# Niema-Lab/AmpliPy

Measured on AMD Instinct MI355X. Metric: aligned reads/s through trim+pileup+call, 30 kb ref @ 10k x depth, higher is better.
Workload: dtype u8/int32

## Files before the change

amplipy_amd/csrc/amp_fast.hpp:

```cpp
#pragma once

#include "amp_tile.hpp"
#include "amp_bf.hpp"

namespace amp {

#ifndef AMP_F_LDSPAD
#define AMP_F_LDSPAD 0
#endif
#ifndef AMP_F4_LEAN
#define AMP_F4_LEAN 1
#endif
#ifndef AMP_F4_BF
#define AMP_F4_BF 1
#endif
__device__ __forceinline__ Bf bf_of(const Cig2 &s) { return Bf{s.a, s.m1, s.k, s.m2, s.c, s.kind, s.op, s.punt ? 1u : 0u}; }
__device__ __forceinline__ Cig2 cig2_of(const Bf &b) { return Cig2{b.op, b.a, b.m1, b.k, b.m2, b.c, b.kind, b.punt != 0u}; }
constexpr int F_NP = 10;
constexpr int F_MAXLEN = 152;
constexpr int F_PW = 256;
#ifndef AMP_F_REPS
#define AMP_F_REPS 8
#endif
constexpr int F_REP = AMP_F_REPS;
// ... 198 lines not shown
    const uint32_t se1 = __builtin_amdgcn_perm(0x00000010u, 0x00080018u, (sq.y >> 4) & 0x07070707u);
    const uint32_t so1 = __builtin_amdgcn_perm(0x00000010u, 0x00080018u, sq.y & 0x07070707u);
    const uint32_t f0 = nibble_to_bytes(m, 0), f1 = nibble_to_bytes(m, 1), f2 = nibble_to_bytes(m, 2), f3 = nibble_to_bytes(m, 3);
    const uint32_t wb = wrep + (inwin ? (uint32_t)d0 * 4u + (((uint32_t)d0 & 1u) ? ooff : 0u) : 0u);
#define F_SH(d, sh, js, v, jv) "v_lshlrev_b32_sdwa " d ", " sh ", " v " dst_sel:DWORD dst_unused:UNUSED_PAD src0_sel:BYTE_" #js " src1_sel:BYTE_" #jv "\n\t"
#define F_AQ(t, off) "ds_add_u64 %0, " t " offset:" #off "\n\t"
    asm volatile(F_SH("v252", "%1", 0, "%5", 0) F_SH("v253", "%2", 0, "%5", 1) F_AQ("v[252:253]", 0)
                 F_SH("v254", "%1", 1, "%5", 2) F_SH("v255", "%2", 1, "%5", 3) F_AQ("v[254:255]", 8)
                 F_SH("v252", "%1", 2, "%6", 0) F_SH("v253", "%2", 2, "%6", 1) F_AQ("v[252:253]", 16)
                 F_SH("v254", "%1", 3, "%6", 2) F_SH("v255", "%2", 3, "%6", 3) F_AQ("v[254:255]", 24)
                 F_SH("v252", "%3", 0, "%7", 0) F_SH("v253", "%4", 0, "%7", 1) F_AQ("v[252:253]", 32)
                 F_SH("v254", "%3", 1, "%7", 2) F_SH("v255", "%4", 1, "%7", 3) F_AQ("v[254:255]", 40)
                 F_SH("v252", "%3", 2, "%8", 0) F_SH("v253", "%4", 2, "%8", 1) F_AQ("v[252:253]", 48)
                 F_SH("v254", "%3", 3, "%8", 2) F_SH("v255", "%4", 3, "%8", 3) "ds_add_u64 %0, v[254:255] offset:56"
                 : : "v"(wb), "v"(se0), "v"(so0), "v"(se1), "v"(so1), "v"(f0), "v"(f1), "v"(f2), "v"(f3) : "memory", "v252", "v253", "v254", "v255");
#undef F_SH
#undef F_AQ
    return redo ? 1u : 0u;
}
__device__ __forceinline__ uint32_t range_bits16(int32_t klo, int32_t khi) {
    klo = klo < 0 ? 0 : (klo > 16 ? 16 : klo); khi = khi > 16 ? 16 : (khi < 0 ? 0 : khi);
    return ((1u << khi) - 1u) & ~((1u << klo) - 1u);
}

#if defined(AMP_DEV) && (!defined(AMP_ABL) || defined(AMP_ABL_STAMPS))
#define F_DBG_PARAM , uint32_t *f_dbg
#define F_GLOB ++f_glob
#define F_EPIW(k) do { __builtin_amdgcn_s_waitcnt(0x4F74); f_epw[0] = wall_clock64(); __builtin_amdgcn_s_waitcnt(0x0F7A); f_epw[1] = wall_clock64(); __builtin_amdgcn_s_waitcnt(0); f_ep[k] = wall_clock64(); } while (0)
#define F_EPI(k) do { __builtin_amdgcn_s_waitcnt(0); f_ep[k] = wall_clock64(); } while (0)
#define F_DBG_ARG(x) , (x)
#define F_STAMP_DECL unsigned long long f_t[8] = {0, 0, 0, 0, 0, 0, 0, 0}, f_prev = __builtin_amdgcn_s_memtime(); const unsigned long long f_k0 = f_prev, f_w0 = wall_clock64(); unsigned long long f_ep[3] = {0, 0, 0}, f_epw[2] = {0, 0}; uint32_t f_glob = 0
#define F_STAMP(k) do { __builtin_amdgcn_sched_barrier(0); __builtin_amdgcn_s_waitcnt(0xC07F); unsigned long long f_n = __builtin_amdgcn_s_memtime(); f_t[k] += f_n - f_prev; f_prev = f_n; __builtin_amdgcn_sched_barrier(0); } while (0)
#define F_STAMP_VM(k) do { __builtin_amdgcn_sched_barrier(0); __builtin_amdgcn_s_waitcnt(0x0070); unsigned long long f_n = __builtin_amdgcn_s_memtime(); f_t[k] += f_n - f_prev; f_prev = f_n; __builtin_amdgcn_sched_barrier(0); } while (0)
#define F_STAMP_OUT do { f_t[0] = __builtin_amdgcn_s_memtime() - f_k0; const unsigned long long f_w1 = wall_clock64(); f_t[7] = f_w1 - f_w0; if (lane == 0) { for (int k = 0; k < 8; ++k) atomicAdd(&ctr[CTR_PHASE0 + k], f_t[k]); \
    atomicMax(&ctr[CTR_STAMP0], f_t[7]); atomicMax(&ctr[CTR_STAMP0 + 1], ~f_t[7]); atomicMax(&ctr[CTR_STAMP0 + 2], ~f_w0); atomicMax(&ctr[CTR_STAMP0 + 3], f_w1); \
    if (f_dbg && wave == 0) { uint32_t *f_o = f_dbg + blockIdx.x * 8; f_o[0] = (uint32_t)f_t[7]; f_o[1] = (uint32_t)f_w0; for (int k = 1; k < 7; ++k) f_o[1 + k] = (uint32_t)(f_t[k] >> 4); } \
    if (f_dbg) { uint32_t *f_o = f_dbg + F_DBG_WAVE0 + (blockIdx.x * F_WAVES + wave) * F_DBG_WAVEWORDS; f_o[0] = (uint32_t)((f_t[1] + f_t[2] + f_t[3] + f_t[4] + f_t[5] + f_t[6]) >> 4); f_o[1] = (uint32_t)(f_epw[0] - f_w0); f_o[2] = (uint32_t)(f_epw[1] - f_epw[0]); f_o[3] = (uint32_t)(f_ep[0] - f_epw[1]); f_o[4] = (uint32_t)(f_ep[1] - f_ep[0]); f_o[5] = (uint32_t)(f_ep[2] - f_ep[1]); } } } while (0)
#else
#define F_DBG_PARAM
#define F_DBG_ARG(x)
#define F_GLOB
#define F_EPIW(k)
#define F_EPI(k)
#define F_STAMP_DECL
#define F_STAMP(k)
#define F_STAMP_VM(k)
#define F_STAMP_OUT
#endif

#define F_ARGS \
    const int32_t *a_pos, int32_t a_min_quality, const uint16_t *a_flag, int32_t a_window, const int32_t *a_tlen, int32_t a_do_trim, \
    const uint32_t *a_lseq, int32_t a_do_count, const uint32_t *a_cig_off32, int32_t a_ref_len, const uint32_t *a_cig, int32_t a_max_primer_len, \
    const uint32_t *a_seq_off8, int32_t reads_per_block, const uint8_t *a_seq, int32_t a_epoch, const uint8_t *a_qual, int32_t pad1, \
    const int32_t *a_min_start, int32_t pad2, const int32_t *a_max_end, int32_t pad3, \
    int32_t *a_new_pos, int32_t pad4, uint32_t *a_new_ncig, int32_t pad5, uint32_t *a_new_cig, int32_t pad6, int32_t *a_o_ref_len, int32_t pad7, \
    uint8_t *a_trim_flags, int32_t pad8, uint8_t *a_status, int32_t pad9, \
    uint32_t *counts, int32_t pad10, amp_ins_event *a_ev, int32_t pad11, unsigned long long *a_ctr, int32_t pad12, uint32_t *a_ins_at, int32_t pad13, \
    uint32_t *glist, int32_t pad14, uint32_t *gcnt, int32_t pad15, \
    int64_t a_n_reads, int32_t pad17, uint64_t read_base, int32_t pad18, long long a_ev_cap
#define F_ARGS_PASS(P, rd, out, eb, rpb) \
    (rd).pos, (P).min_quality, (rd).flag, (P).window, (rd).tlen, (P).do_trim, (rd).lseq, (P).do_count, (rd).cig_off32, (P).ref_len, (rd).cig, \
    (P).max_primer_len, (rd).seq_off8, (rpb), (rd).seq, (int32_t)(P).epoch, (rd).qual, 0, (P).min_start, 0, (P).max_end, 0, (out).new_pos, 0, (out).new_ncig, 0, \
    (out).new_cig, 0, (out).ref_len, 0, (out).trim_flags, 0, (out).status, 0, counts, 0, (eb).ev, 0, (eb).ctr, 0, (eb).ins_at, 0, glist, 0, gcnt, 0, \
    (rd).n_reads, 0, read_base, 0, (eb).cap

#if AMP_F_ADD64
#define F_COUNT5(sq, m, d0, lim, wr) count_piece5q(sq, m, d0, lim, wr, (uint32_t)(F_REPW * 4))
#else
#define F_COUNT5(sq, m, d0, lim, wr) count_piece5(sq, m, d0, lim, wr)
#endif
template <int W>
__global__ void __launch_bounds__(F_WAVES * 64, 2)
k_fast(F_ARGS F_DBG_PARAM) {
    const KParams P{a_min_quality, a_window, a_do_trim, a_do_count, a_ref_len, a_max_primer_len, a_min_start, a_max_end, (uint32_t)a_epoch};
    const amp_dev_reads rd{a_n_reads, a_pos, a_flag, a_tlen, a_lseq, a_cig_off32, a_cig, a_seq_off8, a_seq, a_qual, 0, 0};
    const DevOut out{a_new_pos, a_new_ncig, a_new_cig, a_o_ref_len, a_trim_flags, a_status};
    const EventBuf eb{a_ev, a_ctr, a_ins_at, a_ev_cap};
    __shared__ uint4 s_stage[F_WAVES][(F_PAD + F_STAGE + 16) / 16];
    __shared__ __attribute__((aligned(8))) uint32_t s_pwin[F_WAVES][F_REP * F_REPW];
    __shared__ uint32_t s_bwin[F_BPL * F_BW];
    __shared__ uint32_t s_ticket, s_gcur;
#if AMP_F_LDSPAD > 0
    __shared__ uint32_t s_pad[AMP_F_LDSPAD / 4];
    if (P.ref_len == -12345) s_pad[threadIdx.x] = 1;
#endif
    unsigned long long *const ctr = eb.ctr;
    const int tid = threadIdx.x, wave = tid >> 6, lane = tid & 63;
    F_STAMP_DECL;
    const int64_t n = rd.n_reads;
    const int64_t rb = (int64_t)blockIdx.x * reads_per_block;
    const int64_t re = rb + reads_per_block < n ? rb + reads_per_block : n;
    lds_u32 *const bwin = (lds_u32 *)s_bwin;
    lds_u32 *const pwin = (lds_u32 *)s_pwin[wave];
    for (int i = tid; i < F_BPL * F_BW; i += F_WAVES * 64) bwin[i] = 0;
    for (int i = lane; i < F_REP * F_REPW; i += 64) pwin[i] = 0;
    if (lane < F_PAD / 4) ((lds_u32 *)s_stage[wave])[lane] = 0x11111111u;
    if (tid == 0) { s_ticket = 0; s_gcur = 0; }
    if (tid == 0 && blockIdx.x == 0) { eb.ctr[CTR_LONG_N] = 0ull; eb.ctr[CTR_LONG_TICKET] = 0ull; eb.ctr[CTR_GEN_LEFT] = 0ull; }
    int32_t bw_base = rb < n ? rd.pos[rb] : 0;
    bw_base = (bw_base < 16 ? 0 : bw_base - 16) & ~15;
    __syncthreads();

    const int32_t mq = P.min_quality;
    const uint32_t mqc = (uint32_t)(mq > 256 ? 256 : mq);
    const uint32_t thr = mqc * (uint32_t)W;
    const uint32_t mqb = (uint32_t)mq * 0x01010101u;
    const uint32_t G = (uint32_t)P.ref_len;
    const uint32_t n_tb = re > rb ? (uint32_t)((re - rb + 63) / 64) : 0u;
    auto take_ticket = [&]() {
        uint32_t t = 0;
        if (lane == 0) t = __hip_atomic_fetch_add((lds_u32 *)&s_ticket, 1u, __ATOMIC_RELAXED, __HIP_MEMORY_SCOPE_WORKGROUP);
        return (uint32_t)__builtin_amdgcn_readfirstlane((int)t);
    };
    const int64_t wend = re;
    unsigned long long n_err = 0;
#ifndef AMP_F_REPSHIFT
#define AMP_F_REPSHIFT 2
#endif
    const uint32_t rep = (F_REP & (F_REP - 1)) ? ((uint32_t)lane >> AMP_F_REPSHIFT) % (uint32_t)F_REP : ((uint32_t)lane >> AMP_F_REPSHIFT) & (uint32_t)(F_REP - 1);
    const uint32_t phi_lane = ((uint32_t)lane >> 1) & 1u ? 8u : 0u;
#if AMP_F_ADD64
    lds_u8 *const wrep = (lds_u8 *)pwin + (rep & (uint32_t)(F_REP / 2 - 1)) * (uint32_t)(2 * F_REPW * 4);
    static_assert((F_REP & 1) == 0 && (F_REPW & 1) == 1, "two arrays per replica, the second one an odd number of words behind the first");
#else
    lds_u8 *const wrep = (lds_u8 *)pwin + rep * (uint32_t)(F_REPW * 4);
#endif
    lds_u8 *const stage = (lds_u8 *)s_stage[wave] + F_PAD;
    int32_t pw_base = 0;
    int pw_tiles = F_FLUSH;
    const unsigned ev_shard = blockIdx.x & (EV_SHARDS - 1);
    amp_ins_event *const ev_list = eb.ev + (size_t)ev_shard * (size_t)eb.cap;
    unsigned long long ev_base = 0;
    uint32_t ev_left = 0;

    auto fold = [&]() {
        asm volatile("s_waitcnt lgkmcnt(0)" ::: "memory");
        wave_sync();
#pragma unroll 1
        for (int idx = lane; idx < F_PW; idx += 64) {
            uint32_t ag = 0, ct = 0;
#pragma unroll
            for (int r = 0; r < F_REP; ++r) {
                const uint32_t w = pwin[r * F_REPW + idx];
                pwin[r * F_REPW + idx] = 0;
                ag += w & 0x00FF00FFu; ct += (w >> 8) & 0x00FF00FFu;
            }
            if (ag | ct) {
                const int32_t p = pw_base + idx;
                const uint32_t d = (uint32_t)(p - bw_base);
                const uint32_t c4[4] = {ag & 0xFFFFu, ct & 0xFFFFu, ag >> 16, ct >> 16};
#pragma unroll
                for (int c = 0; c < 4; ++c) {
                    if (!c4[c]) continue;
                    if (d < (uint32_t)F_BW) lds_add(bwin + c * F_BW + d, c4[c]);
                    else if ((uint32_t)p < G) { atomicAdd(&counts[(size_t)p * AMP_NSYM + c], c4[c]); F_GLOB; }
                }
            }
        }
        wave_sync();
    };
    auto pad_events = [&]() {
        if ((uint32_t)lane < ev_left && (long long)(ev_base + (unsigned)lane) < eb.cap) ev_list[ev_base + (unsigned)lane] = amp_ins_event{-1, 0u, 0, 0};
    };

    struct Hdr { int32_t pos, tlen; uint32_t lseq, flag, c0, c1, o8; };
    struct HdrP { int32_t pos; uint32_t lf, c0, o8;
        __device__ uint32_t lseq() const { return lf & 0xFFFFu; }
        __device__ uint32_t nops() const { return (lf >> 19) & 7u; }
        __device__ uint32_t flag() const { return ((lf >> 16) & 1u) | (((lf >> 17) & 1u) << 4); }
        __device__ bool isize_flag() const { return (lf >> 18) & 1u; } };
    auto pack_hdr = [&](const Hdr &h) {
        const uint32_t n = h.c1 - h.c0, at = (uint32_t)(h.tlen < 0 ? -(int64_t)h.tlen : (int64_t)h.tlen);
        const bool isz = ((int64_t)at - P.max_primer_len) > (int64_t)h.lseq;
        return HdrP{h.pos, (h.lseq > 0xFFFFu ? 0xFFFFu : h.lseq) | ((h.flag & 1u) << 16) | (((h.flag >> 4) & 1u) << 17) | ((isz ? 1u : 0u) << 18) | ((n > 7u ? 7u : n) << 19),
                    h.c0, h.o8};
    };
    struct Cg { uint32_t w[5]; };
    struct Geo { uint32_t np, phi, row, Tq; int ntake; bool solo, taken, fastq; };
    struct Tabs { int32_t L, R; };
    struct Bytes { uint4 raws[F_STAGE / 2048]; };
    struct Shape { Cig2 s; bool ok; int32_t refspan; };
    auto load_hdr = [&](int64_t t0) {
        Hdr h{0, 0, 0u, 0u, 0u, 0u, 0u};
        const int64_t i = t0 + lane;
        if (i < wend) {
            h.pos = rd.pos[i]; h.flag = rd.flag[i]; h.tlen = rd.tlen[i]; h.lseq = rd.lseq[i];
            h.c0 = rd.cig_off32[i]; h.c1 = rd.cig_off32[i + 1]; h.o8 = rd.seq_off8[i];
        }
        return h;
    };
    auto load_cig = [&](const HdrP &h) {
        Cg c{{0u, 0u, 0u, 0u, 0u}};
        const uint32_t nops = h.nops();
        if (nops >= 1u && nops <= 5u) {
#pragma unroll
            for (uint32_t k = 0; k < 5u; ++k) c.w[k] = rd.cig[h.c0 + (k < nops ? k : 0u)];
        }
        return c;
    };
    auto geometry = [&](const HdrP &h, int64_t t0, uint32_t &m0) {
        Geo g;
        const bool valid = t0 + lane < wend;
        const uint32_t hl = h.lseq();
        const bool shortq = valid && hl >= 1u && hl <= (uint32_t)F_MAXLEN;
        g.phi = shortq ? phi_lane : 0u;
        g.np = shortq ? (hl + g.phi + 15u) >> 4 : 1u;
        m0 = __builtin_amdgcn_readfirstlane(h.o8);
        g.row = (h.o8 - m0) * 8u;
        const uint32_t nch = (hl + 7u) >> 3;
        const bool fits = valid && h.o8 >= m0 && (h.o8 - m0) <= (uint32_t)(F_STAGE / 8) &&
                          g.row + 8u * nch + (shortq ? 8u : 0u) <= (uint32_t)F_STAGE;
        const unsigned long long fitmask = __ballot(fits);
        g.ntake = fitmask == ~0ull ? 64 : __builtin_ctzll(~fitmask);
        g.solo = g.ntake == 0;
        if (g.solo) g.ntake = 1;
        g.taken = lane < g.ntake && !g.solo;
        g.Tq = g.solo ? 0u : (uint32_t)__builtin_amdgcn_readlane((int)(g.row + 8u * nch), g.ntake - 1);
        g.fastq = g.taken && shortq;
        return g;
    };
    auto shape_of = [&](const HdrP &h, const Cg &c, bool fastq) {
        Shape r;
#if AMP_F4_BF
        bool ok;
        r.s = cig2_of(bf_from_words5((int)h.nops(), c.w[0], c.w[1], c.w[2], c.w[3], c.w[4], (int32_t)h.lseq(), F_MAXINS, F_MAXDEL, ok));
        r.ok = ok & fastq;
        if (!r.ok) r.s = Cig2{0u, 0, 0, 0, 0, 0, 0, false};
#else
        r.s = Cig2{0u, 0, 0, 0, 0, 0, 0, false};
        const int nops = (int)h.nops();
        r.ok = fastq && nops >= 1 && nops <= 5 && cig2_from_words5(nops, c.w, (int32_t)h.lseq(), r.s);
        if (r.ok && ((r.s.kind == 1 && r.s.k > F_MAXINS) || (r.s.kind == 2 && r.s.k > F_MAXDEL))) r.ok = false;
        if (!r.ok) r.s = Cig2{0u, 0, 0, 0, 0, 0, 0, false};
#endif
        r.refspan = r.ok ? r.s.m1 + r.s.m2 + (r.s.kind == 2 ? r.s.k : 0) : 1;
        return r;
    };
    auto load_tabs = [&](const HdrP &h, const Shape &sh) {
        Tabs t{-1, -1};
        const bool in_ref = (uint32_t)h.pos < G && (uint32_t)(h.pos + sh.refspan - 1) < G;
        if (sh.ok && P.do_trim && in_ref) { t.L = P.max_end[h.pos]; t.R = P.min_start[h.pos + sh.refspan - 1]; }
        return t;
    };
    auto issue_bytes = [&](const Geo &g, uint32_t m0) {
        Bytes x;
        const uint8_t *qrun = rd.qual + (int64_t)m0 * 8;
        const uint8_t *srun = rd.seq + (int64_t)m0 * 4;
        const uint32_t lastq = g.Tq ? (g.Tq - 1u) & ~15u : 0u, lasts = g.Tq ? ((g.Tq >> 1) - 1u) & ~15u : 0u;
#pragma unroll
        for (int sl = 0; sl < F_STAGE / 1024; ++sl) {
            uint32_t off = (uint32_t)(sl * 1024 + lane * 16);
            off = off < lastq ? off : lastq;
            __builtin_amdgcn_global_load_lds((const __attribute__((address_space(1))) void *)(qrun + off),
                                             (__attribute__((address_space(3))) void *)(stage + sl * 1024), 16, 0, 0);
        }
#pragma unroll
        for (int sl = 0; sl < F_STAGE / 2048; ++sl) {
            uint32_t off = (uint32_t)(sl * 1024 + lane * 16);
            off = off < lasts ? off : lasts;
            const uint32_t *sp = (const uint32_t *)(srun + off);
            x.raws[sl] = make_uint4(sp[0], sp[1], sp[2], sp[3]);
        }
        return x;
    };
    enum : uint32_t { P_STORED = 1u << 24, P_LIST = 1u << 25, P_STATUS_ONLY = 1u << 26 };
    struct Pend { uint32_t i, slot_lo; int32_t pos, reflen; uint32_t meta, cw0, cw1, cw2, cw3, cw4; };
    Pend pend{0u, 0u, 0, 0, 0u, 0u, 0u, 0u, 0u, 0u};
    auto store_pending = [&](const Pend &r) {
#if defined(AMP_DEV) && defined(AMP_ABL)
        if (AMP_ABL & 8) return;
#endif
        const uint32_t ncig = r.meta & 0xFFu;
        if (r.meta & P_STORED) {
            uint32_t *home = out.new_cig + ((size_t)r.slot_lo + 3 * (size_t)r.i);
            if (ncig > 0u) home[0] = r.cw0;
            if (ncig > 1u) home[1] = r.cw1;
            if (ncig > 2u) home[2] = r.cw2;
            if (ncig > 3u) home[3] = r.cw3;
            if (ncig > 4u) home[4] = r.cw4;
            if (out.new_pos) out.new_pos[r.i] = r.pos;
            if (out.new_ncig) out.new_ncig[r.i] = ncig;
            if (out.ref_len) out.ref_len[r.i] = r.reflen;
            if (out.trim_flags) out.trim_flags[r.i] = (uint8_t)(r.meta >> 16);
            if (out.status) out.status[r.i] = (uint8_t)(r.meta >> 8);
        }
        const bool has = (r.meta & P_LIST) != 0;
        const unsigned long long m = __ballot(has);
        if (m) {
            uint32_t base = 0;
            if (lane == 0) base = __hip_atomic_fetch_add((lds_u32 *)&s_gcur, (uint32_t)__popcll(m), __ATOMIC_RELAXED, __HIP_MEMORY_SCOPE_WORKGROUP);
            base = (uint32_t)__builtin_amdgcn_readfirstlane((int)base);
            if (has) glist[(size_t)rb + base + __popcll(m & ((1ull << lane) - 1ull))] = r.i | ((r.meta & P_STATUS_ONLY) ? GL_STATUS_ONLY : 0u);
        }
    };

    uint32_t pw_lim = 0;
    auto count_piece = [&](const uint4 &q, const uint2 &sq, int32_t j0, int32_t qa_, int32_t qb_, int32_t dbase_) -> bool {
        return fast_count_piece(q, sq, j0, qa_, qb_, dbase_, mqb, pw_lim, (uint32_t)(uintptr_t)wrep);
    };

#ifndef AMP_F_STAGGER
#define AMP_F_STAGGER 4000
#endif
    if (AMP_F_STAGGER > 0) {
        const unsigned long long t_end = __builtin_amdgcn_s_memtime() + (unsigned long long)AMP_F_STAGGER * (unsigned)wave;
        while (__builtin_amdgcn_s_memtime() < t_end) __builtin_amdgcn_s_sleep(8);
    }
    uint32_t tkN = take_ticket(), tkN2 = 0;
    int64_t i0 = rb, i1 = rb + 64 * (int64_t)tkN, i2 = rb;
    int tile_no = 0; (void)tile_no;
    HdrP hN = pack_hdr(load_hdr(i1));
    Hdr hN2{0, 0, 0u, 0u, 0u, 0u, 0u};
    Cg cN = load_cig(hN);
    uint32_t m0N = 0;
    Geo gN = geometry(hN, i1, m0N);
    Bytes xN = issue_bytes(gN, m0N);
    tkN2 = take_ticket();
    i2 = rb + 64 * (int64_t)tkN2;
    hN2 = load_hdr(i2);
    while (tkN < n_tb) {
        __builtin_amdgcn_s_waitcnt(0x0F70);
        F_STAMP(1);
#if defined(AMP_DEV) && defined(AMP_ABL)
        if (AMP_ABL & 32) { if (((tile_no++) + (wave >> 2)) & 1) __builtin_amdgcn_s_setprio(1); else __builtin_amdgcn_s_setprio(0); }
#endif
        const HdrP h = hN;
        const Cg cA = cN;
        const Geo g = gN;
        const Bytes xA = xN;
        hN = pack_hdr(hN2);
        i0 = i1; i1 = i2; tkN = tkN2;
        const int64_t i = i0 + lane;
        const int32_t pos = h.pos;
        const uint32_t lseq = h.lseq(), flag = h.flag(), c0 = h.c0, o8 = h.o8;
        const uint32_t np = g.np, phi = g.phi;
        const bool solo = g.solo, taken = g.taken, fastq = g.fastq;
        const Shape shp = shape_of(h, cA, fastq);
        const Tabs tA = load_tabs(h, shp);
        {
            const int32_t first_pos = __builtin_amdgcn_readfirstlane(pos);
            const int32_t want = (first_pos < 16 ? 0 : first_pos - 16) & ~15;
            if (pw_tiles >= F_FLUSH || want < pw_base || want - pw_base >= 64) {
                if (pw_tiles) fold();
                pw_base = want; pw_tiles = 0;
            }
            ++pw_tiles;
        }
        pw_lim = (int64_t)G - pw_base >= (int64_t)F_PW ? (uint32_t)F_PW : (uint32_t)(G > (uint32_t)pw_base ? G - (uint32_t)pw_base : 0u);
        const uint32_t rot = (uint32_t)lane % np;
        const uint8_t *qrow = rd.qual + (int64_t)o8 * 8;
        const uint8_t *srow = rd.seq + (int64_t)o8 * 4;
        const int32_t lrow = fastq ? (int32_t)g.row - (int32_t)phi : 0;
        const lds_u8 *const lq = stage + (fastq ? (int32_t)g.row : 0);
        uint4 q16[F_NP];
        uint2 s8[F_NP];
        wave_sync();
#pragma unroll
        for (int k = 0; k < F_NP; ++k) {
            uint32_t p = (uint32_t)k + rot;
            p = p >= np ? p - np : p;
            p = (uint32_t)k < np ? p : np - 1u;
            const lds_u8 *src = stage + lrow + (int32_t)(p * 16u);
            const amp_u32x2 a = *(const lds_u32x2 *)src, b = *(const lds_u32x2 *)(src + 8);
            q16[k] = make_uint4(a.x, a.y, b.x, b.y);
        }
        Cig2 s = shp.s;
        const bool shaped = shp.ok;
        const bool in_ref = (uint32_t)pos < G && (uint32_t)(pos + shp.refspan - 1) < G;
        const bool rev = (flag & 0x10u) != 0;
        const int32_t q_ins = s.kind ? s.a + s.m1 : 0, q_seg2 = q_ins + (s.kind == 1 ? s.k : 0);
        TrimState ts{pos, 1, 0u, 0};
#if AMP_F4_BF
        {
            const bool trim = shaped & (P.do_trim != 0), use = trim & in_ref;
            ts.err = (trim & !in_ref) ? AMP_RS_INDEX_REF : 0;
            int32_t p2 = pos; uint32_t f2 = 0u;
            const Bf sp = bf_trim_primers(bf_of(s), p2, f2, flag, h.isize_flag(), (int32_t)lseq, tA.L, tA.R);
            s = cig2_of(bf_pick(use, sp, bf_of(s))); ts.pos = use ? p2 : pos; ts.flags = use ? f2 : 0u;
        }
        const bool scan = shaped & (P.do_trim != 0) & (ts.err == 0) & !s.punt;
        int32_t lo, qlen;
        bf_quality_window(bf_of(s), (int32_t)lseq, lo, qlen);
        lo = scan ? lo + (int32_t)phi : 0; qlen = scan ? qlen : 0;
#else
        if (shaped && P.do_trim) {
            if (!in_ref) ts.err = AMP_RS_INDEX_REF;
            else cig2_trim_primers_isize(ts, flag, h.isize_flag(), (int32_t)lseq, s, tA.L, tA.R);
        }
        const bool scan = shaped && P.do_trim && !ts.err && !s.punt;
        int32_t lo = 0, qlen = 0;
        if (scan) { cig2_quality_window(s, (int32_t)lseq, lo, qlen); lo += (int32_t)phi; }
#endif
        const int32_t hi = lo + qlen;
        const int32_t first = !scan ? 0 : ((rev || qlen < W) ? lo : lo + qlen - W + 1) - (int32_t)phi;
        const int32_t tab = first & ~7, g_ins = q_ins & ~7, g_b = q_seg2 & ~7;
        const amp_u32x2 tw0 = *(const lds_u32x2 *)(lq + tab), tw1 = *(const lds_u32x2 *)(lq + tab + 8);
        const amp_u32x2 iq0 = *(const lds_u32x2 *)(lq + g_ins), iq1 = *(const lds_u32x2 *)(lq + g_ins + 8);
        const amp_u32x2 bq0 = *(const lds_u32x2 *)(lq + g_b), bq1 = *(const lds_u32x2 *)(lq + g_b + 8);
        wave_sync();
#pragma unroll
        for (int sl = 0; sl < F_STAGE / 2048; ++sl) *(lds_u32x4 *)(stage + sl * 1024 + lane * 16) = amp_u32x4{xA.raws[sl].x, xA.raws[sl].y, xA.raws[sl].z, xA.raws[sl].w};
        wave_sync();
#if AMP_F4_LEAN
        {
            if (lane == 0) *(lds_u32x4 *)(stage + ((g.Tq >> 1) & ~3u)) = amp_u32x4{0x11111111u, 0x11111111u, 0x11111111u, 0x11111111u};
            wave_sync();
            const uint32_t e = fastq ? lseq & 7u : 0u;
            if (e) {
                lds_u32 *w = (lds_u32 *)(stage + (g.row >> 1) + 4u * (lseq >> 3));
                const uint32_t x = *w, xs = ((x & 0x0F0F0F0Fu) << 4) | ((x >> 4) & 0x0F0F0F0Fu);
                const uint32_t keepn = (1u << (4u * e)) - 1u;
                const uint32_t ys = (xs & keepn) | (0x11111111u & ~keepn);
                *w = ((ys & 0x0F0F0F0Fu) << 4) | ((ys >> 4) & 0x0F0F0F0Fu);
            }
            wave_sync();
        }
#endif
#pragma unroll
        for (int k = 0; k < F_NP; ++k) {
            uint32_t p = (uint32_t)k + rot;
            p = p >= np ? p - np : p;
            p = (uint32_t)k < np ? p : np - 1u;
            const lds_u8 *src = stage + (lrow >> 1) + (int32_t)(p * 8u);
            s8[k] = make_uint2(*(const lds_u32 *)src, *(const lds_u32 *)(src + 4));
        }
        const lds_u8 *const lsq = stage + (fastq ? (int32_t)(g.row >> 1) : 0) + (g_b >> 1);
        const uint2 bsq = make_uint2(*(const lds_u32 *)lsq, *(const lds_u32 *)(lsq + 4));
        wave_sync();
        store_pending(pend);
        tkN2 = take_ticket();
        i2 = rb + 64 * (int64_t)tkN2;
        cN = load_cig(hN);
        gN = geometry(hN, i1, m0N);
        xN = issue_bytes(gN, m0N);
        hN2 = load_hdr(i2);
        F_STAMP(2);

        int32_t ffmin = 0x7FFFFFFF, lemax = -1;
#if defined(AMP_DEV) && defined(AMP_ABL)
        if (P.do_trim && !(AMP_ABL & 4)) {
#else
        if (P.do_trim) {
#endif
#pragma unroll
            for (int k = 0; k < F_NP; ++k) {
                uint32_t p = (uint32_t)k + rot;
                p = p >= np ? p - np : p;
                p = (uint32_t)k < np ? p : np;
                const int32_t j0 = (int32_t)(p * 16u);
                uint2 nx = make_uint2(q16[0].x, q16[0].y);
                if (k + 1 < F_NP && (uint32_t)(k + 1) < np) nx = make_uint2(q16[k + 1].x, q16[k + 1].y);
                uint32_t fail = piece_fail_bits<W>(q16[k], nx, thr);
                int32_t blo = lo - j0, bhi = hi - W - j0;
                blo = blo < 0 ? 0 : (blo > 16 ? 16 : blo); bhi = bhi > 15 ? 15 : (bhi < -1 ? -1 : bhi);
                fail &= (0xFFFFu >> (15 - bhi)) & (0xFFFFu << blo);
                const int32_t f1 = j0 + (__builtin_ffs((int)fail) - 1), e1 = j0 + (31 - __builtin_clz(fail)) + W;
                ffmin = fail && f1 < ffmin ? f1 : ffmin;
                lemax = fail && e1 > lemax ? e1 : lemax;
            }
        }

        F_STAMP(3);
        bool general = i < re && !shaped;
        bool stored = false;
        uint32_t ncig = 0, cw[5] = {0u, 0u, 0u, 0u, 0u};
        int32_t reflen = 0;
        if (shaped) {
            uint32_t fb = phi ? q16[0].z : q16[0].x;
            const uint32_t slot0 = rot ? np - rot : 0u;
#pragma unroll
            for (int k = 1; k < F_NP; ++k) fb = ((uint32_t)k == slot0) ? (phi ? q16[k].z : q16[k].x) : fb;
            if ((fb & 0xFFu) == 0xFFu || s.punt) {
                general = true;
            } else {
                if (scan) {
                    int32_t iq;
                    if (!rev && ffmin != 0x7FFFFFFF) iq = ffmin - lo;
                    else if (rev && lemax >= 0) iq = lemax - lo;
                    else {
                        iq = rev ? 0 : qlen;
                        int32_t acc = 0;
                        const uint64_t t_lo = (uint64_t)tw0.x | ((uint64_t)tw0.y << 32), t_hi = (uint64_t)tw1.x | ((uint64_t)tw1.y << 32);
                        const int32_t kmax = qlen < W - 1 ? qlen : W - 1;
                        const int32_t qlo = lo - (int32_t)phi, qhi = hi - (int32_t)phi;
                        for (int32_t k = 1; k <= kmax; ++k) {
                            const uint32_t o = (uint32_t)((rev ? qlo + k - 1 : qhi - k) - tab);
                            acc += (int32_t)(((o < 8u ? t_lo : t_hi) >> ((o & 7u) * 8u)) & 0xFFu);
                            if ((int64_t)acc < (int64_t)mq * k) iq = rev ? k : qlen - k;
                        }
                    }
#if AMP_F4_BF
                    { uint32_t f2 = ts.flags; s = cig2_of(bf_trim_quality(bf_of(s), ts.pos, f2, rev, iq, qlen)); ts.flags = f2; }
#else
                    cig2_trim_quality(ts, rev, iq, qlen, s);
#endif
                }
                if (s.punt) {
                    general = true;
                } else {
                    if (!ts.err) {
                        const uint32_t part[5] = {((uint32_t)s.a << 4) | OP_S, ((uint32_t)s.m1 << 4) | s.op,
                                                  ((uint32_t)s.k << 4) | (s.kind == 1 ? OP_I : OP_D), ((uint32_t)s.m2 << 4) | s.op,
                                                  ((uint32_t)s.c << 4) | OP_S};
                        const bool has[5] = {s.a > 0, s.m1 > 0, s.kind != 0, s.kind != 0 && s.m2 > 0, s.c > 0};
#pragma unroll
                        for (int t = 0; t < 5; ++t) {
                            if (has[t]) {
#pragma unroll
                                for (int j = 0; j < 5; ++j) cw[j] = ncig == (uint32_t)j ? part[t] : cw[j];
                                ++ncig;
                            }
                        }
                        reflen = s.ref_len();
                    }
                    stored = true;
                    if (ts.err) ++n_err;
                }
            }
        }
        const bool counted = stored && !ts.err && P.do_count;
        F_STAMP(4);
        const bool two = counted && s.kind != 0;
        const int32_t qa1 = counted ? s.a + (int32_t)phi : 0, qb1 = counted ? qa1 + s.m1 : 0;
        const int32_t qa2 = two ? qb1 + (s.kind == 1 ? s.k : 0) : qb1, qb2 = two ? qa2 + s.m2 : qa2;
        const int32_t pos2 = ts.pos + s.m1 + (s.kind == 2 ? s.k : 0);
        bool bad_extra = false;
        if (two && s.kind == 2) {
            for (int32_t j = 0; j < s.k; ++j) {
                const int32_t r = ts.pos + s.m1 + j;
                const uint32_t d = (uint32_t)(r - bw_base);
                if ((uint32_t)r >= G) bad_extra = true;
                else if (d < (uint32_t)F_BW) lds_add_nt(bwin + 4 * F_BW + d, 1u);
                else atomicAdd(&counts[(size_t)r * AMP_NSYM + 5], 1u);
            }
        }
        {
            uint32_t good = 0;
            if (two && s.kind == 1) {
                const uint32_t o0 = ok_bits4(iq0.x, mqb) >> 7, o1 = ok_bits4(iq0.y, mqb) >> 7, o2 = ok_bits4(iq1.x, mqb) >> 7, o3 = ok_bits4(iq1.y, mqb) >> 7;
                auto nib = [](uint32_t o) { return ((o * 0x00204081u) >> 21) & 0xFu; };
                const uint32_t m16 = nib(o0) | (nib(o1) << 4) | (nib(o2) << 8) | (nib(o3) << 12);
                good = (m16 >> (uint32_t)(s.a + s.m1 - g_ins)) & ((1u << s.k) - 1u);
            }
            uint32_t runs = good & ~(good << 1);
            const unsigned long long em = __ballot(runs != 0u);
            if (em) {
                const uint32_t total = (uint32_t)__popcll(em);
                if (total > ev_left) {
                    pad_events();
                    unsigned long long nb = 0;
                    if (lane == 0) nb = atomicAdd(&ctr[CTR_EV_SHARD0 + ev_shard], (unsigned long long)F_EVGRAN);
                    ev_base = __shfl(nb, 0); ev_left = F_EVGRAN;
                }
                if (runs) {
                    const int32_t q0 = s.a + s.m1, r2 = ts.pos + s.m1, ref_end = ts.pos + s.m1 + s.m2;
                    const unsigned long long slot = ev_base + (unsigned)__popcll(em & ((1ull << lane) - 1ull));
                    const uint32_t rid = (uint32_t)(read_base + (uint64_t)i);
                    bool firstrun = true;
                    while (runs) {
                        const int32_t js = __builtin_ctz(runs);
                        runs &= runs - 1u;
                        const int32_t je = js + __builtin_ctz(~(good >> js));
                        int32_t elo, ehi;
                        if (je == s.k && s.m2 > 0 && r2 == 0) py_slice(q0 + js, q0 + je + 1, (int32_t)lseq, elo, ehi);
                        else py_slice(q0 + js - 1, q0 + je, (int32_t)lseq, elo, ehi);
                        int32_t ins_pos = je == s.k ? r2 : ref_end;
                        ins_pos = ins_pos - 1 > 0 ? ins_pos - 1 : 0;
                        const bool inside = (uint32_t)ins_pos < G;
                        if (!inside) bad_extra = true;
                        if (firstrun) {
                            if ((long long)slot < eb.cap) ev_list[slot] = inside ? amp_ins_event{ins_pos, rid, elo, ehi} : amp_ins_event{-1, 0u, 0, 0};
                            if (inside) {
                                const uint32_t d = (uint32_t)(ins_pos - bw_base);
                                if (d < (uint32_t)F_BW) lds_add_nt(bwin + 5 * F_BW + d, 1u);
                                else atomicAdd(&eb.ins_at[ins_pos], 1u);
                            }
                        } else if (inside) {
                            eb.record(ins_pos, rid, elo, ehi);
                        }
                        firstrun = false;
                    }
                }
                ev_base += total; ev_left -= total;
            }
        }
        uint32_t redo = 0;
#if AMP_F4_LEAN
        uint32_t okm[F_NP];
#pragma unroll
        for (int k = 0; k < F_NP; ++k) okm[k] = ok_bits16(q16[k], mqb);
        const uint32_t okB = ok_bits16(make_uint4(bq0.x, bq0.y, bq1.x, bq1.y), mqb);
#endif
        int32_t xbe = 0, jb = 0;
        bool has_b = false;
        if (two) {
            const int32_t jstar = (qb1 - 1) & ~15;
            has_b = jstar + 16 > qa2 && qb2 > qa2;
            xbe = qb2 < jstar + 16 ? qb2 : jstar + 16;
            jb = g_b + (int32_t)phi;
        }
        const int32_t end_pos = two ? pos2 + s.m2 : ts.pos + s.m1;
        bool todo = counted;
#if defined(AMP_DEV) && defined(AMP_ABL)
        if (AMP_ABL & 2) todo = false;
// ... 25 lines not shown
#endif
#pragma unroll
            for (int k = 0; k < F_NP; ++k) {
                uint32_t p = (uint32_t)k + rot;
                p = p >= np ? p - np : p;
                p = (uint32_t)k < np ? p : np;
                const int32_t j0 = (int32_t)(p * 16u);
                const bool second = j0 >= qb1;
#if AMP_F4_LEAN
                redo |= F_COUNT5(s8[k], okm[k] & range_bits16((second ? a2 : a1) - j0, (second ? b2 : b1) - j0), (second ? dbase2 : dbase1) + j0, lim16,
                                 (uint32_t)(uintptr_t)wrep) << k;
#else
                asm volatile("" : "+v"(q16[k].x), "+v"(q16[k].y), "+v"(q16[k].z), "+v"(q16[k].w), "+v"(s8[k].x), "+v"(s8[k].y));
                if (count_piece(q16[k], s8[k], j0, second ? a2 : a1, second ? b2 : b1, second ? dbase2 : dbase1)) redo |= 1u << k;
                __builtin_amdgcn_sched_barrier(0);
#endif
            }
            todo = todo && !now;
        }
        F_STAMP(5);
        bool want_status = bad_extra;
        if (__ballot(redo != 0u)) {
            if (redo) {
                const int32_t a1 = qa1 - (int32_t)phi, b1 = qb1 - (int32_t)phi, a2 = qa2 - (int32_t)phi, b2 = qb2 - (int32_t)phi;
                auto careful = [&](int32_t x0, int32_t x1, int32_t qa_q, int32_t rp0) {
                    for (int32_t q = x0; q < x1; ++q) {
                        if ((int32_t)qrow[q] < mq) continue;
                        const uint32_t sb = srow[q >> 1];
                        const uint32_t col = col_of_code((q & 1) ? (sb & 15u) : (sb >> 4));
                        const int32_t rp = rp0 + (q - qa_q);
                        const uint32_t d = (uint32_t)(rp - bw_base);
                        if (col > 4u || (uint32_t)rp >= G) want_status = true;
                        else if (d < (uint32_t)F_BW && col < (uint32_t)F_NPL) lds_add_nt(bwin + col * F_BW + d, 1u);
                        else atomicAdd(&counts[(size_t)rp * AMP_NSYM + col], 1u);
                    }
                };
                for (int k = 0; k < F_NP; ++k) {
                    if (!((redo >> k) & 1u)) continue;
                    uint32_t p = (uint32_t)k + rot;
                    p = p >= np ? p - np : p;
                    const int32_t j0 = (int32_t)(p * 16u) - (int32_t)phi;
                    const bool second = j0 + (int32_t)phi >= qb1;
                    const int32_t sa = second ? a2 : a1, sb_ = second ? b2 : b1;
                    careful(j0 < sa ? sa : j0, j0 + 16 < sb_ ? j0 + 16 : sb_, sa, second ? pos2 : ts.pos);
                }
                if ((redo >> F_NP) & 1u) careful(a2, xbe - (int32_t)phi, a2, pos2);
            }
        }

        {
            uint32_t meta = ncig | ((uint32_t)ts.err << 8) | ((ts.err ? 0u : ts.flags) << 16) | (stored ? P_STORED : 0u);
            if (general) meta |= P_LIST;
            else if (counted && want_status) meta |= P_LIST | P_STATUS_ONLY;
            pend = Pend{(uint32_t)i, c0, ts.pos, reflen, meta, cw[0], cw[1], cw[2], cw[3], cw[4]};
        }
        F_STAMP(6);
    }
    F_EPIW(0);
    store_pending(pend);
    pad_events();
    F_EPI(1);
    if (pw_tiles && n_tb) fold();
    F_EPI(2);
    asm volatile("s_waitcnt lgkmcnt(0)" ::: "memory");
    __syncthreads();
#if defined(AMP_DEV) && defined(AMP_ABL)
    if (AMP_ABL & 16) return;
#endif
    for (int i = tid; i < F_BPL * F_BW; i += F_WAVES * 64) {
        const uint32_t v = bwin[i];
        if (v) {
            const int pl = i / F_BW, d = i - pl * F_BW;
            const uint32_t p = (uint32_t)(bw_base + d);
            if (p < G) {
                if (pl < F_NPL) atomicAdd(&counts[(size_t)p * AMP_NSYM + pl], v);
                else if (pl == 4) atomicAdd(&counts[(size_t)p * AMP_NSYM + 5], v);
                else atomicAdd(&eb.ins_at[p], v);
            }
        }
    }
    if (n_err) atomicAdd(&ctr[CTR_ERROR_READS], n_err);
    F_STAMP_OUT;
    if (tid == 0) { gcnt[blockIdx.x] = s_gcur; if (s_gcur) eb.ctr[CTR_EPOCH] = (unsigned long long)P.epoch; }
}

__global__ void __launch_bounds__(256)
k_gcompact(const uint32_t *__restrict__ glist, const uint32_t *__restrict__ gcnt, int reads_per_block, int64_t n_reads,
           uint32_t *__restrict__ dense, GenGeo *geo, uint32_t gen_grid, unsigned long long *ctr,
           const uint32_t *__restrict__ cig_off32, uint32_t *__restrict__ llist, uint32_t *__restrict__ lpos, int long_max_ops) {
    __shared__ uint32_t s_part[4], s_lw[4], s_lbase;
    const int tid = threadIdx.x;
    uint32_t acc = 0;
    for (int b = tid; b < (int)blockIdx.x; b += 256) acc += gcnt[b];
    for (int o = 32; o > 0; o >>= 1) acc += __shfl_down(acc, o);
    if ((tid & 63) == 0) s_part[tid >> 6] = acc;
    __syncthreads();
    const uint32_t off = s_part[0] + s_part[1] + s_part[2] + s_part[3];
    const uint32_t cnt = gcnt[blockIdx.x];
    const int64_t sbeg = (int64_t)blockIdx.x * reads_per_block;
    const uint32_t *src = glist + (sbeg < n_reads ? sbeg : 0);
    for (uint32_t k = tid; k < cnt; k += 256) dense[off + k] = src[k];
    if (long_max_ops) {
        const auto kind = [&](uint32_t k) -> uint32_t {
            if (k >= cnt) return 0u;
            const uint32_t e = src[k];
            if (e & GL_STATUS_ONLY) return 0u;
            const uint32_t i = e & GL_INDEX_MASK, nops = cig_off32[i + 1] - cig_off32[i];
            if ((int)nops > long_max_ops) return 0u;
            return (int)nops + 3 > T_MAXOPS ? 1u : 2u;
        };
        uint32_t strict = 0, elig = 0;
        for (uint32_t k = tid; k < cnt; k += 256) { const uint32_t kd = kind(k); strict += kd == 1u ? 1u : 0u; elig += kd ? 1u : 0u; }
        for (int o = 32; o > 0; o >>= 1) { strict += __shfl_down(strict, o); elig += __shfl_down(elig, o); }
        __syncthreads();
        if ((tid & 63) == 0) { s_lw[tid >> 6] = strict; s_part[tid >> 6] = elig; }
        __syncthreads();
// ... 56 lines not shown
```

Baseline: 10.15 billion.

## Load rarely-used kernel arguments lazily from kernarg segment to cut SGPR pressure

Replaces the up-front loading of many output and event-buffer pointer arguments with on-demand scalar loads from the kernarg segment at fixed offsets, so they do not stay live in SGPRs across the main loop. The first header load is also moved ahead of the wave-stagger sleep. The first-base lookup is simplified to a single LDS read, and the trim selection is simplified to apply unconditionally when trimming is enabled. The hard-coded kernarg offsets depend on the argument layout and break silently if the signature changes, and the repeated scalar loads add latency at each use site.

Result: faster. 10.36 billion, median of 6 (+2.1%).

```diff
diff --git a/amplipy_amd/csrc/amp_fast.hpp b/amplipy_amd/csrc/amp_fast.hpp
--- a/amplipy_amd/csrc/amp_fast.hpp
+++ b/amplipy_amd/csrc/amp_fast.hpp
@@ -254,7 +254,7 @@
 #define F_STAMP_DECL unsigned long long f_t[8] = {0, 0, 0, 0, 0, 0, 0, 0}, f_prev = __builtin_amdgcn_s_memtime(); const unsigned long long f_k0 = f_prev, f_w0 = wall_clock64(); unsigned long long f_ep[3] = {0, 0, 0}, f_epw[2] = {0, 0}; uint32_t f_glob = 0
 #define F_STAMP(k) do { __builtin_amdgcn_sched_barrier(0); __builtin_amdgcn_s_waitcnt(0xC07F); unsigned long long f_n = __builtin_amdgcn_s_memtime(); f_t[k] += f_n - f_prev; f_prev = f_n; __builtin_amdgcn_sched_barrier(0); } while (0)
 #define F_STAMP_VM(k) do { __builtin_amdgcn_sched_barrier(0); __builtin_amdgcn_s_waitcnt(0x0070); unsigned long long f_n = __builtin_amdgcn_s_memtime(); f_t[k] += f_n - f_prev; f_prev = f_n; __builtin_amdgcn_sched_barrier(0); } while (0)
-#define F_STAMP_OUT do { f_t[0] = __builtin_amdgcn_s_memtime() - f_k0; const unsigned long long f_w1 = wall_clock64(); f_t[7] = f_w1 - f_w0; if (lane == 0) { for (int k = 0; k < 8; ++k) atomicAdd(&ctr[CTR_PHASE0 + k], f_t[k]); \
+#define F_STAMP_OUT do { f_t[0] = __builtin_amdgcn_s_memtime() - f_k0; const unsigned long long f_w1 = wall_clock64(); f_t[7] = f_w1 - f_w0; if (lane == 0) { unsigned long long *const ctr = late_ctr(); for (int k = 0; k < 8; ++k) atomicAdd(&ctr[CTR_PHASE0 + k], f_t[k]); \
     atomicMax(&ctr[CTR_STAMP0], f_t[7]); atomicMax(&ctr[CTR_STAMP0 + 1], ~f_t[7]); atomicMax(&ctr[CTR_STAMP0 + 2], ~f_w0); atomicMax(&ctr[CTR_STAMP0 + 3], f_w1); \
     if (f_dbg && wave == 0) { uint32_t *f_o = f_dbg + blockIdx.x * 8; f_o[0] = (uint32_t)f_t[7]; f_o[1] = (uint32_t)f_w0; for (int k = 1; k < 7; ++k) f_o[1 + k] = (uint32_t)(f_t[k] >> 4); } \
     if (f_dbg) { uint32_t *f_o = f_dbg + F_DBG_WAVE0 + (blockIdx.x * F_WAVES + wave) * F_DBG_WAVEWORDS; f_o[0] = (uint32_t)((f_t[1] + f_t[2] + f_t[3] + f_t[4] + f_t[5] + f_t[6]) >> 4); f_o[1] = (uint32_t)(f_epw[0] - f_w0); f_o[2] = (uint32_t)(f_epw[1] - f_epw[0]); f_o[3] = (uint32_t)(f_ep[0] - f_epw[1]); f_o[4] = (uint32_t)(f_ep[1] - f_ep[0]); f_o[5] = (uint32_t)(f_ep[2] - f_ep[1]); } } } while (0)
@@ -286,6 +286,22 @@
     (out).new_cig, 0, (out).ref_len, 0, (out).trim_flags, 0, (out).status, 0, counts, 0, (eb).ev, 0, (eb).ctr, 0, (eb).ins_at, 0, glist, 0, gcnt, 0, \
     (rd).n_reads, 0, read_base, 0, (eb).cap
 
+enum : uint32_t { KA_MIN_START = 144, KA_MAX_END = 160, KA_NEW_POS = 176, KA_NEW_NCIG = 192, KA_NEW_CIG = 208, KA_O_REF_LEN = 224, KA_TRIM_FLAGS = 240,
+                  KA_STATUS = 256, KA_COUNTS = 272, KA_EV = 288, KA_CTR = 304, KA_INS_AT = 320, KA_GLIST = 336, KA_GCNT = 352, KA_N_READS = 368,
+                  KA_READ_BASE = 384, KA_EV_CAP = 400 };
+template <typename T>
+__device__ __forceinline__ T karg_late(uint32_t off) {
+    static_assert(sizeof(T) == 8, "the late-loaded arguments are pointers and 64-bit values");
+    asm volatile("" : "+s"(off));
+    const unsigned long long v = *(const __attribute__((address_space(4))) unsigned long long *)
+        ((const __attribute__((address_space(4))) uint8_t *)__builtin_amdgcn_kernarg_segment_ptr() + off);
+    return __builtin_bit_cast(T, v);
+}
+template <typename T>
+__device__ __forceinline__ T *karg_late_ptr(uint32_t off) {
+    return (T *)karg_late<__attribute__((address_space(1))) T *>(off);
+}
+
 #if AMP_F_ADD64
 #define F_COUNT5(sq, m, d0, lim, wr) count_piece5q(sq, m, d0, lim, wr, (uint32_t)(F_REPW * 4))
 #else
@@ -294,10 +310,10 @@
 template <int W>
 __global__ void __launch_bounds__(F_WAVES * 64, 2)
 k_fast(F_ARGS F_DBG_PARAM) {
-    const KParams P{a_min_quality, a_window, a_do_trim, a_do_count, a_ref_len, a_max_primer_len, a_min_start, a_max_end, (uint32_t)a_epoch};
+    const KParams P{a_min_quality, a_window, a_do_trim, a_do_count, a_ref_len, a_max_primer_len, nullptr, nullptr, (uint32_t)a_epoch};
     const amp_dev_reads rd{a_n_reads, a_pos, a_flag, a_tlen, a_lseq, a_cig_off32, a_cig, a_seq_off8, a_seq, a_qual, 0, 0};
-    const DevOut out{a_new_pos, a_new_ncig, a_new_cig, a_o_ref_len, a_trim_flags, a_status};
-    const EventBuf eb{a_ev, a_ctr, a_ins_at, a_ev_cap};
+    auto late_ctr = [] { return karg_late_ptr<unsigned long long>(KA_CTR); };
+    auto late_eb = [] { return EventBuf{karg_late_ptr<amp_ins_event>(KA_EV), karg_late_ptr<unsigned long long>(KA_CTR), karg_late_ptr<uint32_t>(KA_INS_AT), karg_late<long long>(KA_EV_CAP)}; };
     __shared__ uint4 s_stage[F_WAVES][(F_PAD + F_STAGE + 16) / 16];
     __shared__ __attribute__((aligned(8))) uint32_t s_pwin[F_WAVES][F_REP * F_REPW];
     __shared__ uint32_t s_bwin[F_BPL * F_BW];
@@ -306,7 +322,6 @@
     __shared__ uint32_t s_pad[AMP_F_LDSPAD / 4];
     if (P.ref_len == -12345) s_pad[threadIdx.x] = 1;
 #endif
-    unsigned long long *const ctr = eb.ctr;
     const int tid = threadIdx.x, wave = tid >> 6, lane = tid & 63;
     F_STAMP_DECL;
     const int64_t n = rd.n_reads;
@@ -318,7 +333,7 @@
     for (int i = lane; i < F_REP * F_REPW; i += 64) pwin[i] = 0;
     if (lane < F_PAD / 4) ((lds_u32 *)s_stage[wave])[lane] = 0x11111111u;
     if (tid == 0) { s_ticket = 0; s_gcur = 0; }
-    if (tid == 0 && blockIdx.x == 0) { eb.ctr[CTR_LONG_N] = 0ull; eb.ctr[CTR_LONG_TICKET] = 0ull; eb.ctr[CTR_GEN_LEFT] = 0ull; }
+    if (tid == 0 && blockIdx.x == 0) { unsigned long long *const ctr = late_ctr(); ctr[CTR_LONG_N] = 0ull; ctr[CTR_LONG_TICKET] = 0ull; ctr[CTR_GEN_LEFT] = 0ull; }
     int32_t bw_base = rb < n ? rd.pos[rb] : 0;
     bw_base = (bw_base < 16 ? 0 : bw_base - 16) & ~15;
     __syncthreads();
@@ -351,7 +366,6 @@
     int32_t pw_base = 0;
     int pw_tiles = F_FLUSH;
     const unsigned ev_shard = blockIdx.x & (EV_SHARDS - 1);
-    amp_ins_event *const ev_list = eb.ev + (size_t)ev_shard * (size_t)eb.cap;
     unsigned long long ev_base = 0;
     uint32_t ev_left = 0;
 
@@ -375,14 +389,17 @@
                 for (int c = 0; c < 4; ++c) {
                     if (!c4[c]) continue;
                     if (d < (uint32_t)F_BW) lds_add(bwin + c * F_BW + d, c4[c]);
-                    else if ((uint32_t)p < G) { atomicAdd(&counts[(size_t)p * AMP_NSYM + c], c4[c]); F_GLOB; }
+                    else if ((uint32_t)p < G) { atomicAdd(&karg_late_ptr<uint32_t>(KA_COUNTS)[(size_t)p * AMP_NSYM + c], c4[c]); F_GLOB; }
                 }
             }
         }
         wave_sync();
     };
     auto pad_events = [&]() {
-        if ((uint32_t)lane < ev_left && (long long)(ev_base + (unsigned)lane) < eb.cap) ev_list[ev_base + (unsigned)lane] = amp_ins_event{-1, 0u, 0, 0};
+        if ((uint32_t)lane < ev_left) {
+            const EventBuf eb = late_eb();
+            if ((long long)(ev_base + (unsigned)lane) < eb.cap) eb.ev[(size_t)ev_shard * (size_t)eb.cap + ev_base + (unsigned)lane] = amp_ins_event{-1, 0u, 0, 0};
+        }
     };
 
     struct Hdr { int32_t pos, tlen; uint32_t lseq, flag, c0, c1, o8; };
@@ -445,9 +462,8 @@
         Shape r;
 #if AMP_F4_BF
         bool ok;
-        r.s = cig2_of(bf_from_words5((int)h.nops(), c.w[0], c.w[1], c.w[2], c.w[3], c.w[4], (int32_t)h.lseq(), F_MAXINS, F_MAXDEL, ok));
-        r.ok = ok & fastq;
-        if (!r.ok) r.s = Cig2{0u, 0, 0, 0, 0, 0, 0, false};
+        r.s = cig2_of(bf_from_words5((int)h.nops(), c.w[0], c.w[1], c.w[2], c.w[3], c.w[4], fastq ? (int32_t)h.lseq() : 0, F_MAXINS, F_MAXDEL, ok));
+        r.ok = ok;
 #else
         r.s = Cig2{0u, 0, 0, 0, 0, 0, 0, false};
         const int nops = (int)h.nops();
@@ -458,10 +474,10 @@
         r.refspan = r.ok ? r.s.m1 + r.s.m2 + (r.s.kind == 2 ? r.s.k : 0) : 1;
         return r;
     };
-    auto load_tabs = [&](const HdrP &h, const Shape &sh) {
+    auto load_tabs = [&](const HdrP &h, const Shape &sh, bool trim) {
         Tabs t{-1, -1};
         const bool in_ref = (uint32_t)h.pos < G && (uint32_t)(h.pos + sh.refspan - 1) < G;
-        if (sh.ok && P.do_trim && in_ref) { t.L = P.max_end[h.pos]; t.R = P.min_start[h.pos + sh.refspan - 1]; }
+        if (trim && in_ref) { t.L = karg_late_ptr<const int32_t>(KA_MAX_END)[h.pos]; t.R = karg_late_ptr<const int32_t>(KA_MIN_START)[h.pos + sh.refspan - 1]; }
         return t;
     };
     auto issue_bytes = [&](const Geo &g, uint32_t m0) {
@@ -494,6 +510,8 @@
 #endif
         const uint32_t ncig = r.meta & 0xFFu;
         if (r.meta & P_STORED) {
+            const DevOut out{karg_late_ptr<int32_t>(KA_NEW_POS), karg_late_ptr<uint32_t>(KA_NEW_NCIG), karg_late_ptr<uint32_t>(KA_NEW_CIG),
+                             karg_late_ptr<int32_t>(KA_O_REF_LEN), karg_late_ptr<uint8_t>(KA_TRIM_FLAGS), karg_late_ptr<uint8_t>(KA_STATUS)};
             uint32_t *home = out.new_cig + ((size_t)r.slot_lo + 3 * (size_t)r.i);
             if (ncig > 0u) home[0] = r.cw0;
             if (ncig > 1u) home[1] = r.cw1;
@@ -512,7 +530,7 @@
             uint32_t base = 0;
             if (lane == 0) base = __hip_atomic_fetch_add((lds_u32 *)&s_gcur, (uint32_t)__popcll(m), __ATOMIC_RELAXED, __HIP_MEMORY_SCOPE_WORKGROUP);
             base = (uint32_t)__builtin_amdgcn_readfirstlane((int)base);
-            if (has) glist[(size_t)rb + base + __popcll(m & ((1ull << lane) - 1ull))] = r.i | ((r.meta & P_STATUS_ONLY) ? GL_STATUS_ONLY : 0u);
+            if (has) karg_late_ptr<uint32_t>(KA_GLIST)[(size_t)rb + base + __popcll(m & ((1ull << lane) - 1ull))] = r.i | ((r.meta & P_STATUS_ONLY) ? GL_STATUS_ONLY : 0u);
         }
     };
 
@@ -524,14 +542,15 @@
 #ifndef AMP_F_STAGGER
 #define AMP_F_STAGGER 4000
 #endif
+    uint32_t tkN = take_ticket(), tkN2 = 0;
+    int64_t i0 = rb, i1 = rb + 64 * (int64_t)tkN, i2 = rb;
+    const Hdr h_first = load_hdr(i1);
     if (AMP_F_STAGGER > 0) {
         const unsigned long long t_end = __builtin_amdgcn_s_memtime() + (unsigned long long)AMP_F_STAGGER * (unsigned)wave;
         while (__builtin_amdgcn_s_memtime() < t_end) __builtin_amdgcn_s_sleep(8);
     }
-    uint32_t tkN = take_ticket(), tkN2 = 0;
-    int64_t i0 = rb, i1 = rb + 64 * (int64_t)tkN, i2 = rb;
     int tile_no = 0; (void)tile_no;
-    HdrP hN = pack_hdr(load_hdr(i1));
+    HdrP hN = pack_hdr(h_first);
     Hdr hN2{0, 0, 0u, 0u, 0u, 0u, 0u};
     Cg cN = load_cig(hN);
     uint32_t m0N = 0;
@@ -558,7 +577,10 @@
         const uint32_t np = g.np, phi = g.phi;
         const bool solo = g.solo, taken = g.taken, fastq = g.fastq;
         const Shape shp = shape_of(h, cA, fastq);
-        const Tabs tA = load_tabs(h, shp);
+        int32_t do_trim_t = P.do_trim, do_count_t = P.do_count;
+        asm volatile("" : "+s"(do_trim_t), "+s"(do_count_t));
+        const bool trim = shp.ok & (do_trim_t != 0);
+        const Tabs tA = load_tabs(h, shp, trim);
         {
             const int32_t first_pos = __builtin_amdgcn_readfirstlane(pos);
             const int32_t want = (first_pos < 16 ? 0 : first_pos - 16) & ~15;
@@ -594,22 +616,20 @@
         TrimState ts{pos, 1, 0u, 0};
 #if AMP_F4_BF
         {
-            const bool trim = shaped & (P.do_trim != 0), use = trim & in_ref;
             ts.err = (trim & !in_ref) ? AMP_RS_INDEX_REF : 0;
             int32_t p2 = pos; uint32_t f2 = 0u;
-            const Bf sp = bf_trim_primers(bf_of(s), p2, f2, flag, h.isize_flag(), (int32_t)lseq, tA.L, tA.R);
-            s = cig2_of(bf_pick(use, sp, bf_of(s))); ts.pos = use ? p2 : pos; ts.flags = use ? f2 : 0u;
-        }
-        const bool scan = shaped & (P.do_trim != 0) & (ts.err == 0) & !s.punt;
+            s = cig2_of(bf_trim_primers(bf_of(s), p2, f2, flag, h.isize_flag(), (int32_t)lseq, tA.L, tA.R)); ts.pos = p2; ts.flags = f2;
+        }
+        const bool scan = trim & (ts.err == 0) & !s.punt;
         int32_t lo, qlen;
         bf_quality_window(bf_of(s), (int32_t)lseq, lo, qlen);
         lo = scan ? lo + (int32_t)phi : 0; qlen = scan ? qlen : 0;
 #else
-        if (shaped && P.do_trim) {
+        if (trim) {
             if (!in_ref) ts.err = AMP_RS_INDEX_REF;
             else cig2_trim_primers_isize(ts, flag, h.isize_flag(), (int32_t)lseq, s, tA.L, tA.R);
         }
-        const bool scan = shaped && P.do_trim && !ts.err && !s.punt;
+        const bool scan = trim && !ts.err && !s.punt;
         int32_t lo = 0, qlen = 0;
         if (scan) { cig2_quality_window(s, (int32_t)lseq, lo, qlen); lo += (int32_t)phi; }
 #endif
@@ -619,6 +639,7 @@
         const amp_u32x2 tw0 = *(const lds_u32x2 *)(lq + tab), tw1 = *(const lds_u32x2 *)(lq + tab + 8);
         const amp_u32x2 iq0 = *(const lds_u32x2 *)(lq + g_ins), iq1 = *(const lds_u32x2 *)(lq + g_ins + 8);
         const amp_u32x2 bq0 = *(const lds_u32x2 *)(lq + g_b), bq1 = *(const lds_u32x2 *)(lq + g_b + 8);
+        const uint32_t fb = *lq;
         wave_sync();
 #pragma unroll
         for (int sl = 0; sl < F_STAGE / 2048; ++sl) *(lds_u32x4 *)(stage + sl * 1024 + lane * 16) = amp_u32x4{xA.raws[sl].x, xA.raws[sl].y, xA.raws[sl].z, xA.raws[sl].w};
@@ -660,9 +681,9 @@
 
         int32_t ffmin = 0x7FFFFFFF, lemax = -1;
 #if defined(AMP_DEV) && defined(AMP_ABL)
-        if (P.do_trim && !(AMP_ABL & 4)) {
+        if (do_trim_t && !(AMP_ABL & 4)) {
 #else
-        if (P.do_trim) {
+        if (do_trim_t) {
 #endif
 #pragma unroll
             for (int k = 0; k < F_NP; ++k) {
@@ -688,11 +709,7 @@
         uint32_t ncig = 0, cw[5] = {0u, 0u, 0u, 0u, 0u};
         int32_t reflen = 0;
         if (shaped) {
-            uint32_t fb = phi ? q16[0].z : q16[0].x;
-            const uint32_t slot0 = rot ? np - rot : 0u;
-#pragma unroll
-            for (int k = 1; k < F_NP; ++k) fb = ((uint32_t)k == slot0) ? (phi ? q16[k].z : q16[k].x) : fb;
-            if ((fb & 0xFFu) == 0xFFu || s.punt) {
+            if (fb == 0xFFu || s.punt) {
                 general = true;
             } else {
                 if (scan) {
@@ -729,7 +746,7 @@
                         for (int t = 0; t < 5; ++t) {
                             if (has[t]) {
 #pragma unroll
-                                for (int j = 0; j < 5; ++j) cw[j] = ncig == (uint32_t)j ? part[t] : cw[j];
+                                for (int j = (t == 3 ? 1 : 0); j <= t; ++j) cw[j] = ncig == (uint32_t)j ? part[t] : cw[j];
                                 ++ncig;
                             }
                         }
@@ -740,7 +757,7 @@
                 }
             }
         }
-        const bool counted = stored && !ts.err && P.do_count;
+        const bool counted = stored && !ts.err && do_count_t;
         F_STAMP(4);
         const bool two = counted && s.kind != 0;
         const int32_t qa1 = counted ? s.a + (int32_t)phi : 0, qb1 = counted ? qa1 + s.m1 : 0;
@@ -753,7 +770,7 @@
                 const uint32_t d = (uint32_t)(r - bw_base);
                 if ((uint32_t)r >= G) bad_extra = true;
                 else if (d < (uint32_t)F_BW) lds_add_nt(bwin + 4 * F_BW + d, 1u);
-                else atomicAdd(&counts[(size_t)r * AMP_NSYM + 5], 1u);
+                else atomicAdd(&karg_late_ptr<uint32_t>(KA_COUNTS)[(size_t)r * AMP_NSYM + 5], 1u);
             }
         }
         {
@@ -771,13 +788,14 @@
                 if (total > ev_left) {
                     pad_events();
                     unsigned long long nb = 0;
-                    if (lane == 0) nb = atomicAdd(&ctr[CTR_EV_SHARD0 + ev_shard], (unsigned long long)F_EVGRAN);
+                    if (lane == 0) nb = atomicAdd(&late_ctr()[CTR_EV_SHARD0 + ev_shard], (unsigned long long)F_EVGRAN);
                     ev_base = __shfl(nb, 0); ev_left = F_EVGRAN;
                 }
                 if (runs) {
                     const int32_t q0 = s.a + s.m1, r2 = ts.pos + s.m1, ref_end = ts.pos + s.m1 + s.m2;
                     const unsigned long long slot = ev_base + (unsigned)__popcll(em & ((1ull << lane) - 1ull));
-                    const uint32_t rid = (uint32_t)(read_base + (uint64_t)i);
+                    const uint32_t rid = (uint32_t)(karg_late<uint64_t>(KA_READ_BASE) + (uint64_t)i);
+                    const EventBuf eb = late_eb();
                     bool firstrun = true;
                     while (runs) {
                         const int32_t js = __builtin_ctz(runs);
@@ -791,7 +809,7 @@
                         const bool inside = (uint32_t)ins_pos < G;
                         if (!inside) bad_extra = true;
                         if (firstrun) {
-                            if ((long long)slot < eb.cap) ev_list[slot] = inside ? amp_ins_event{ins_pos, rid, elo, ehi} : amp_ins_event{-1, 0u, 0, 0};
+                            if ((long long)slot < eb.cap) eb.ev[(size_t)ev_shard * (size_t)eb.cap + slot] = inside ? amp_ins_event{ins_pos, rid, elo, ehi} : amp_ins_event{-1, 0u, 0, 0};
                             if (inside) {
                                 const uint32_t d = (uint32_t)(ins_pos - bw_base);
                                 if (d < (uint32_t)F_BW) lds_add_nt(bwin + 5 * F_BW + d, 1u);
@@ -883,7 +901,7 @@
                         const uint32_t d = (uint32_t)(rp - bw_base);
                         if (col > 4u || (uint32_t)rp >= G) want_status = true;
                         else if (d < (uint32_t)F_BW && col < (uint32_t)F_NPL) lds_add_nt(bwin + col * F_BW + d, 1u);
-                        else atomicAdd(&counts[(size_t)rp * AMP_NSYM + col], 1u);
+                        else atomicAdd(&karg_late_ptr<uint32_t>(KA_COUNTS)[(size_t)rp * AMP_NSYM + col], 1u);
                     }
                 };
                 for (int k = 0; k < F_NP; ++k) {
@@ -918,21 +936,22 @@
 #if defined(AMP_DEV) && defined(AMP_ABL)
     if (AMP_ABL & 16) return;
 #endif
+    uint32_t *const counts_l = karg_late_ptr<uint32_t>(KA_COUNTS), *const ins_at_l = karg_late_ptr<uint32_t>(KA_INS_AT);
     for (int i = tid; i < F_BPL * F_BW; i += F_WAVES * 64) {
         const uint32_t v = bwin[i];
         if (v) {
             const int pl = i / F_BW, d = i - pl * F_BW;
             const uint32_t p = (uint32_t)(bw_base + d);
             if (p < G) {
-                if (pl < F_NPL) atomicAdd(&counts[(size_t)p * AMP_NSYM + pl], v);
-                else if (pl == 4) atomicAdd(&counts[(size_t)p * AMP_NSYM + 5], v);
-                else atomicAdd(&eb.ins_at[p], v);
+                if (pl < F_NPL) atomicAdd(&counts_l[(size_t)p * AMP_NSYM + pl], v);
+                else if (pl == 4) atomicAdd(&counts_l[(size_t)p * AMP_NSYM + 5], v);
+                else atomicAdd(&ins_at_l[p], v);
             }
         }
     }
-    if (n_err) atomicAdd(&ctr[CTR_ERROR_READS], n_err);
+    if (n_err) atomicAdd(&late_ctr()[CTR_ERROR_READS], n_err);
     F_STAMP_OUT;
-    if (tid == 0) { gcnt[blockIdx.x] = s_gcur; if (s_gcur) eb.ctr[CTR_EPOCH] = (unsigned long long)P.epoch; }
+    if (tid == 0) { karg_late_ptr<uint32_t>(KA_GCNT)[blockIdx.x] = s_gcur; if (s_gcur) late_ctr()[CTR_EPOCH] = (unsigned long long)P.epoch; }
 }
 
 __global__ void __launch_bounds__(256)
```
